# HadrienG2/grayscott

Measured on AMD Instinct MI355X. Metric: Mcells×steps/s and achieved HBM GB/s (% of roofline), 16384² f32 grid, higher is better.
Workload: dtype f32

## Files before the change

grayscott_amd/capi.py:

```python
from __future__ import annotations

import ctypes
import os

_HERE = os.path.dirname(os.path.abspath(__file__))
LIB_PATH = os.environ.get("GS_HIP_LIBRARY") or os.path.join(_HERE, "libgs_hip.so")

GS_OK = 0
GS_ERR_INVALID = -1
GS_ERR_HIP = -2
GS_ERR_RCCL = -3
GS_ERR_NO_DEVICE = -4
GS_ERR_UNSUPPORTED = -5
GS_ERR_NOMEM = -6

GS_MATH_STRICT, GS_MATH_FUSED = 0, 1
GS_KERNEL_AUTO, GS_KERNEL_SIMPLE, GS_KERNEL_STREAM, GS_KERNEL_TB, GS_KERNEL_LDS, GS_KERNEL_TILE, GS_KERNEL_WINDOW = 0, 1, 2, 3, 4, 5, 6
GS_BOUNDARY_CLIPPED, GS_BOUNDARY_ZERO_HALO, GS_BOUNDARY_PERIODIC, GS_BOUNDARY_NEUMANN = 0, 1, 2, 3
GS_UNIQUE_ID_BYTES = 128
GS_REGION_PAIRS_MAX = 1 << 25
GS_REGION_HIST_MAX = 1 << 25
GS_REGION_SPECTRUM_MAX = 1 << 25
GS_REGION_SPECTRUM_RECORDS_MAX = 1 << 27
GS_REGION_COMPONENTS_MAX = 1 << 20
# ... 26 lines not shown
    "gs_field_reduced_shape", "gs_field_download_reduced", "gs_field_download_reduced_async", "gs_field_colormap_reduced",
    "gs_fields_compare", "gs_members_compare", "gs_fields_copy", "gs_members_copy",
    "gs_members_set_active", "gs_members_get_active",
    "gs_members_set_noise", "gs_members_get_noise", "gs_members_clear_noise",
    "gs_fields_morphology", "gs_members_morphology",
    "gs_region_grid", "gs_fields_region_summaries", "gs_fields_region_morphology", "gs_fields_region_correlation",
    "gs_fields_region_histogram", "gs_fields_region_components", "gs_fields_region_compare", "gs_fields_region_spectrum",
    "gs_fields_correlation", "gs_members_correlation",
    "gs_spectrum_tables", "gs_fields_spectrum", "gs_members_spectrum",
    "gs_fields_components", "gs_members_components",
    "gs_field_component_list", "gs_members_component_list", "gs_component_list_view", "gs_component_list_destroy",
    "gs_fields_match", "gs_members_match", "gs_component_match_view", "gs_component_match_destroy",
    "gs_time_stats_create", "gs_time_stats_destroy", "gs_time_stats_reset", "gs_time_stats_accumulate", "gs_time_stats_samples",
    "gs_time_stats_result", "gs_time_stats_download",
    "gs_members_time_stats_create", "gs_members_time_stats_accumulate", "gs_members_time_stats_result",
    "gs_ctx_quiet_stats", "gs_ctx_quiet_edge_stats",
)


class GsError(RuntimeError):

    def __init__(self, code: int, message: str):
        super().__init__(f"gs_hip error {code}: {message}")
        self.code = code
        self.message = message


class GsParams(ctypes.Structure):

    _fields_ = [
        ("w", (ctypes.c_float * 3) * 3),
# ... 157 lines not shown
        "gs_timer_start": (i32, [vp]),
        "gs_timer_stop": (i32, [vp, P(f32)]),
        "gs_ctx_info": (i32, [vp, ctypes.c_char_p, ctypes.c_size_t, P(u64)]),
        "gs_host_alloc": (i32, [P(vp), u64]),
        "gs_host_free": (i32, [vp]),
        "gs_field_download_async": (i32, [vp, vp, vp]),
        "gs_download_wait": (i32, [vp]),
        "gs_ctx_get_tuned": (i32, [vp, u64, u64, P(i32), P(i32), P(i32), P(i32)]),
        "gs_ctx_set_tuned": (i32, [vp, u64, u64, i32, i32, i32, i32]),
        "gs_ctx_comm_info": (i32, [vp, P(i32), P(i32), P(i32)]),
        "gs_field_colormap": (i32, [vp, vp, f32, vp, i32, vp]),
        "gs_ctx_stats": (i32, [vp, P(GsStats)]),
        "gs_ctx_set_pass_timing": (i32, [vp, i32]),
        "gs_ctx_quiet_stats": (i32, [vp, P(u64)]),
        "gs_ctx_quiet_edge_stats": (i32, [vp, P(u64)]),
        "gs_field_mark_written": (i32, [vp, vp]),
        "gs_rccl_selftest": (i32, [i32, u64]),
        "gs_runtime_info": (i32, [i32, ctypes.c_char_p, ctypes.c_size_t]),
        "gs_fields_place": (i32, [vp, P(vp), i32, P(f32), P(f32)]),
        "gs_debug_place_stats": (i32, [vp, P(u64), P(u64)]),
        "gs_download_wait_but": (i32, [vp, i32]),
        "gs_debug_exchange_probe_create": (i32, [i32, i32, i32, u64, P(vp)]),
        "gs_debug_exchange_probe_run": (i32, [vp, P(f32), P(f32)]),
        "gs_debug_exchange_probe_destroy": (i32, [vp]),
        "gs_ensemble_create": (i32, [vp, P(vp), u64, u64, u64]),
        "gs_ensemble_destroy": (i32, [vp, vp]),
        "gs_ensemble_shape": (i32, [vp, P(u64), P(u64), P(u64)]),
        "gs_ensemble_set_params": (i32, [vp, vp, P(GsParams), u64]),
        "gs_ensemble_seed": (i32, [vp, vp]),
        "gs_ensemble_upload": (i32, [vp, vp, u64, u64, vp, vp]),
# ... 104 lines not shown
```

grayscott_amd/csrc/gs_api.cpp:

```cpp
#include "gs_internal.h"

namespace gsi {

bool is_pow2_or_zero(float w)
{
    if (w == 0.0f) return true;
    int e = 0;
    const float m = std::frexp(std::fabs(w), &e);
    return m == 0.5f;
}

int32_t check_math(const gs_params &p, int32_t math)
{
    if (math != GS_MATH_STRICT && math != GS_MATH_FUSED)
        return fail(GS_ERR_INVALID, "unknown math flavour %d", math);
    if (math == GS_MATH_FUSED)
        for (int i = 0; i < 3; ++i)
            for (int j = 0; j < 3; ++j)
                if (!is_pow2_or_zero(p.w[i][j]))
                    return fail(GS_ERR_UNSUPPORTED,
                                "GS_MATH_FUSED needs stencil weights that are 0 or a power of two "
                                "(w[%d][%d] = %g); use GS_MATH_STRICT", i, j, (double)p.w[i][j]);
    return GS_OK;
}
// ... 141 lines not shown
                    at.kind == GS_ATTACH_MAP ? "parameter-map" : (at.kind == GS_ATTACH_MASK ? "domain-mask" : "noise"));
    const char *name = nullptr;
    hipError_t e;
    switch (kernel) {
    case GS_KERNEL_TB:
        if (ctx->quiet.mode > 0 && !fused && at.kind == GS_ATTACH_NONE) {
            gs_ctx::QuietRt &qr = ctx->quiet;
            e = hipSuccess;
            for (int attempt = 0; attempt < 2; ++attempt) {
                GsQuiet q;
                q.in = qr.words + (size_t)qr.in_slot * qr.cap;
                q.out = qr.words + (size_t)(1 - qr.in_slot) * qr.cap;
                q.edge_skips = qr.words + 2 * qr.cap;
                q.skipped = qr.skipped;
                q.mode = qr.mode;
                q.cap = (int64_t)qr.cap;
                q.need = 0;
                q.launched = 0;
                q.edge_launched = 0;
                if (qr.mode == 1 && qr.words)
                    e = hipMemsetAsync(qr.words, 0, 2 * qr.cap * sizeof(uint32_t), stream);
                if (e == hipSuccess) e = gs_launch_tb_strict(a, fuse, stream, &name, at, &q);
                if (e != hipSuccess) break;
                if (q.need > (int64_t)qr.cap && qr.mode == 1) {
                    if (qr.words) {
                        GS_HIP(hipStreamSynchronize(stream));
                        uint64_t sum = 0;
                        GS_TRY(quiet_edge_skips(ctx, &sum));
                        qr.edge_skipped = sum;
                        GS_HIP(hipFree(qr.words));
                        qr.words = nullptr;
                        qr.cap = 0;
                    }
                    GS_HIP(hipMalloc(&qr.words, 3 * (size_t)q.need * sizeof(uint32_t)));
                    GS_HIP(hipMemset(qr.words, 0, 3 * (size_t)q.need * sizeof(uint32_t)));
                    qr.cap = (size_t)q.need;
                    if (!qr.skipped) {
                        GS_HIP(hipMalloc(&qr.skipped, (size_t)kQuietCounters * kQuietCounterStride * sizeof(unsigned long long)));
                        GS_HIP(hipMemset(qr.skipped, 0, (size_t)kQuietCounters * kQuietCounterStride * sizeof(unsigned long long)));
                    }
                    continue;
                }
                if (q.launched > 0) {
                    qr.launched += (uint64_t)q.launched;
                    qr.edge_launched += (uint64_t)q.edge_launched;
                    qr.passes++;
                    if (qr.mode == 3) qr.steady++;
                } else {
                    qr.refused = true;
                }
                break;
            }
            break;
        }
        e = fused ? gs_launch_tb_fused(a, fuse, stream, &name, at) : gs_launch_tb_strict(a, fuse, stream, &name, at);
        break;
    case GS_KERNEL_SIMPLE:
        e = fused ? gs_launch_simple_fused(a, stream, &name, at) : gs_launch_simple_strict(a, stream, &name, at);
        break;
    case GS_KERNEL_STREAM:
// ... 393 lines not shown
        for (int k = 0; k < 2; ++k) {
            if (b.done[k]) (void)hipEventDestroy(b.done[k]);
            if (b.halod[k]) (void)hipEventDestroy(b.halod[k]);
        }
    }
    if (!ctx->slabs.empty() && (ctx->win.words || ctx->win.planes[0] || ctx->win.desc) && hipSetDevice(ctx->slabs[0].device) == hipSuccess) {
        for (auto p : ctx->win.planes)
            if (p) (void)hipFree(p);
        if (ctx->win.words) (void)hipFree(ctx->win.words);
        if (ctx->win.desc) (void)hipFree(ctx->win.desc);
    }
    if (ctx->win.seen) (void)hipHostFree(ctx->win.seen);
    if (!ctx->slabs.empty() && (ctx->quiet.words || ctx->quiet.skipped) && hipSetDevice(ctx->slabs[0].device) == hipSuccess) {
        if (ctx->quiet.words) (void)hipFree(ctx->quiet.words);
        if (ctx->quiet.skipped) (void)hipFree(ctx->quiet.skipped);
    }
    if (ctx->graph_exec) (void)hipGraphExecDestroy(ctx->graph_exec);
    if (ctx->graph) (void)hipGraphDestroy(ctx->graph);
    if (ctx->band_join) (void)hipEventDestroy(ctx->band_join);
    const bool tuning = std::any_of(std::begin(ctx->tuner_of), std::end(ctx->tuner_of),
                                    [](const gs_ctx::TunerState &ts) { return !ts.tunings.empty(); });
    if (tuning && !ctx->slabs.empty() && hipSetDevice(ctx->slabs[0].device) == hipSuccess)
        for (auto &ts : ctx->tuner_of)
            for (auto &t : ts.tunings)
                for (auto e : t.events)
                    if (e) (void)hipEventDestroy(e);
    (void)hipGetLastError();
    delete ctx;
    return GS_OK;
}
// ... 18 lines not shown
                                            "set GS_RCCL_LIBRARY to the transport to use, or run one slab per process");
    }

    int ndev = 0;
    hipError_t e = hipGetDeviceCount(&ndev);
    if (e != hipSuccess || ndev == 0)
        return fail(GS_ERR_NO_DEVICE, "no HIP device available (%s)", hipGetErrorString(e));

    gs_ctx *ctx = new (std::nothrow) gs_ctx();
    if (!ctx) return fail(GS_ERR_NOMEM, "out of host memory");
    if (params) ctx->p = *params; else gs_default_params(&ctx->p);
    if (opts) ctx->o = *opts; else gs_default_options(&ctx->o);
    ctx->rank = rank;
    ctx->world = world;
    ctx->quiet.enabled = gs_env_int("GS_HIP_QUIET_UNITS", 1, 0, 1) != 0;
    int32_t st = check_math(ctx->p, ctx->o.math);
    if (st == GS_OK && ctx->o.cols_per_lane != 0 && ctx->o.cols_per_lane != 1 && ctx->o.cols_per_lane != 2 &&
        ctx->o.cols_per_lane != 4)
        st = fail(GS_ERR_INVALID, "cols_per_lane must be 0 (auto), 1, 2 or 4, not %d", ctx->o.cols_per_lane);
    if (st == GS_OK && (ctx->o.tile_shape < 0 || ctx->o.tile_shape > 3))
        st = fail(GS_ERR_INVALID, "tile_shape must be 0 (auto), 1 (32 x 64), 2 (16 x 64) or 3 (64 x 64), not %d", ctx->o.tile_shape);
    if (st == GS_OK && ctx->o.boundary != GS_BOUNDARY_CLIPPED && ctx->o.boundary != GS_BOUNDARY_ZERO_HALO &&
        ctx->o.boundary != GS_BOUNDARY_PERIODIC && ctx->o.boundary != GS_BOUNDARY_NEUMANN)
        st = fail(GS_ERR_INVALID, "unknown boundary rule %d", ctx->o.boundary);
    if (st == GS_OK && ctx->o.boundary == GS_BOUNDARY_PERIODIC) {
        if (world > 1 || n_local > 1)
            st = fail(GS_ERR_UNSUPPORTED, "the periodic boundary rule needs a single slab in a single process (got %d local "
                                          "slab(s), %d process(es))", n_local < 1 ? 1 : n_local, world);
        else if (ctx->o.kernel == GS_KERNEL_WINDOW || ctx->o.kernel == GS_KERNEL_LDS)
            st = fail(GS_ERR_UNSUPPORTED, "the periodic boundary rule has no form of the %s kernel",
// ... 207 lines not shown
    if (single && fuse > 1 && ctx->o.rows_per_block == 0 && !ctx->o.no_tune && !tuned_shape(ctx, u0, fuse))
        GS_TRY(tune_online(r, fuse));
    const int kk = tuned_shape(ctx, u0, fuse) && ctx->tuner().tuned.k > 0 && ctx->tuner().tuned.k <= fuse ? ctx->tuner().tuned.k : fuse;
    const int V = bands_for(ctx, u0, kk);
    if (ctx->o.use_graph && single && V == 1 && kk > 1) GS_TRY(replay_graph_batches(r, kk));
    gs_ctx::QuietRt &qr = ctx->quiet;
    const gs_params &pp = ctx->p;
    bool quiet = qr.enabled && single && V == 1 && !ctx->o.use_graph && !mapped && kk >= 2 && kk <= 4 &&
                 ctx->o.math == GS_MATH_STRICT && (ctx->o.boundary == GS_BOUNDARY_CLIPPED || ctx->o.boundary == GS_BOUNDARY_ZERO_HALO) &&
                 (ctx->o.kernel == GS_KERNEL_AUTO || ctx->o.kernel == GS_KERNEL_TB || ctx->o.kernel == GS_KERNEL_TILE ||
                  ctx->o.kernel == GS_KERNEL_WINDOW) &&
                 std::isfinite(pp.du) && std::isfinite(pp.dv) && std::isfinite(pp.feed) && std::isfinite(pp.kill) &&
                 std::isfinite(pp.feed + pp.kill) && std::isfinite(pp.dt);
    for (int i = 0; i < 9; ++i) quiet = quiet && std::isfinite(pp.w[i / 3][i % 3]);
    qr.refused = false;
    int quiet_pass = 0;
    const char *full_pass = nullptr;
    while (r.n < steps) {
        const int k = (steps - r.n) >= (uint64_t)kk ? kk : (int)(steps - r.n);
        if (quiet && k == kk && !qr.refused) {
            qr.mode = quiet_pass < 2 ? quiet_pass + 1 : 3;
            qr.in_slot = r.in;
            ++quiet_pass;
        }
        const int32_t st = r.advance(k == kk ? V : 1, k);
        qr.mode = 0;
        GS_TRY(st);
        if (k == kk) full_pass = ctx->last_kernel;
    }
    if (full_pass) ctx->last_kernel = full_pass;
    if (result_slot) *result_slot = r.in;
    return GS_OK;
}

}

// ... 100 lines not shown
int32_t gs_ctx_quiet_edge_stats(gs_ctx *ctx, uint64_t out[3])
{
    if (!ctx || !out) return fail(GS_ERR_INVALID, "null argument");
    GS_TRY(sync_all(ctx));
    out[0] = ctx->quiet.edge_launched;
    out[1] = out[2] = 0;
    if (ctx->quiet.skipped) {
        unsigned long long host[kQuietCounters * kQuietCounterStride];
        GS_HIP(hipSetDevice(ctx->slabs[0].device));
        GS_HIP(hipMemcpy(host, ctx->quiet.skipped, sizeof host, hipMemcpyDeviceToHost));
        for (int i = 0; i < kQuietCounters; ++i) out[2] += host[i * kQuietCounterStride + 2];
    }
    return gsi::quiet_edge_skips(ctx, &out[1]);
}

int32_t gs_ctx_info(const gs_ctx *ctx, char *kernel_name, size_t cap, uint64_t *launches)
{
    if (!ctx) return fail(GS_ERR_INVALID, "null context");
    if (kernel_name && cap) {
        const gs_ctx::Tuned &t = ctx->tuner().tuned;
        if (t.rpu > 0)
            std::snprintf(kernel_name, cap, "%s@%dx%d", ctx->last_kernel, t.rpu, t.split > 0 ? t.split : 1);
        else
            std::snprintf(kernel_name, cap, "%s", ctx->last_kernel);
    }
    if (launches) *launches = ctx->launches;
    return GS_OK;
}

}
// ... 1 lines not shown
```

grayscott_amd/csrc/gs_internal.h:

```cpp
#pragma once
#pragma GCC visibility push(default)
#include "../../include/gs_hip.h"
#pragma GCC visibility pop
#include "gs_kernels.h"
#include "gs_experiments.h"

#include <dlfcn.h>
#include <hip/hip_runtime.h>
#include <rccl/rccl.h>

#include <algorithm>
#include <cmath>
#include <cstdarg>
#include <cstdio>
#include <cstdlib>
#include <cstring>
#include <new>
#include <string>
#include <utility>
#include <vector>

namespace gsi {

extern thread_local std::string g_last_error;
// ... 128 lines not shown
        std::vector<Launch> launched;
        int32_t seq = 0;
        uint64_t fallbacks = 0;
        struct Image { gs_field *f; float *host; int32_t after_seq; int32_t factor; };
        std::vector<Image> images;
        int32_t *seen = nullptr;
    } win;
    int cu_count = 0;
    struct QuietRt {
        bool enabled = true;
        uint32_t *words = nullptr;
        size_t cap = 0;
        unsigned long long *skipped = nullptr;
        int mode = 0;
        int in_slot = 0;
        bool refused = false;
        uint64_t launched = 0, passes = 0, steady = 0;
        uint64_t edge_launched = 0;
        uint64_t edge_skipped = 0;
    } quiet;
    std::vector<struct gs_time_stats *> time_stats;
    struct Attached {
        int kind = GS_ATTACH_NONE;
        gs_field *plane[2] = {nullptr, nullptr};
        uint64_t gen = 0;
        gs_noise noise{};
    } attached;
    bool noisy() const { return attached.kind == GS_ATTACH_NOISE; }
    bool mapped() const { return attached.kind == GS_ATTACH_MAP; }
    bool masked() const { return attached.kind == GS_ATTACH_MASK; }
// ... 129 lines not shown
```

grayscott_amd/csrc/gs_kernels.h:

```cpp
#pragma once
#include <hip/hip_runtime.h>
#include <stdint.h>

constexpr int kGsResidentCells = 1536;
constexpr int kGsTileMaxSteps = 8;

struct GsStepArgs {
    const float *in_u, *in_v;
    float *out_u, *out_v;
    int32_t rows;
    int32_t cols;
    int32_t pitch;
    int32_t ra0, ra1, rb0, rb1;
    int32_t top_present, bottom_present;
    int32_t ghost;
    int32_t rows_per_unit;
    int32_t big_chunks, small_rpu;
    int32_t mid_chunks, tiny_rpu;
    int32_t bot_first;
    int32_t edge_split, edge_chunks;
    int32_t fast;
    int32_t cpl;
    int32_t allow_fair;
    int32_t edge_kinds;
    int32_t fair_from;
    int32_t xcd_m, xcd_first;
    int32_t zero_halo;
    float w[3][3];
    float du, dv, feed, feed_plus_kill, dt;
};
struct GsMapPlanes {
    const float *feed, *fpk;
};
struct GsMaskPlanes {
    const float *link;
};
constexpr uint32_t kQuietRest = 1, kQuietActive = 2;
constexpr int kQuietCounters = 64, kQuietCounterStride = 16;
struct GsQuiet {
    const uint32_t *in;
    uint32_t *out;
    uint32_t *edge_skips;
    unsigned long long *skipped;
    int32_t mode;
    int32_t pad;
    int64_t cap, need, launched, edge_launched;
};
struct GsNoiseArgs {
    uint32_t key[4];
    float sigma_u, sigma_v;
    uint32_t row0;
    uint32_t pad;
};
enum { GS_ATTACH_NONE = 0, GS_ATTACH_MAP = 1, GS_ATTACH_MASK = 2, GS_ATTACH_NOISE = 3, GS_ATTACH_KINDS = 4 };
struct GsAttached {
    int kind = GS_ATTACH_NONE;
    const float *plane[2] = {nullptr, nullptr};
    GsNoiseArgs noise = {};
};

constexpr int kGsWindowMaxNbr = 14;
// ... 220 lines not shown
```

grayscott_amd/csrc/gs_march.h:

```cpp
#pragma once

namespace {

__host__ __device__ constexpr int tb_sacrificial_lanes(int k, int cpl) { return (k + cpl - 1) / cpl; }
__host__ __device__ constexpr int tb_cols_per_wave(int k, int cpl) { return (64 - 2 * tb_sacrificial_lanes(k, cpl)) * cpl; }
static_assert(tb_cols_per_wave(4, 4) == 248 && tb_cols_per_wave(4, 1) == 56 && tb_cols_per_wave(3, 2) == 120, "");

template <int CPL>
struct RowQ {
    float u[CPL], v[CPL];
};
template <int CPL>
struct RowT {
    float u[CPL + 2], v[CPL + 2];
};

__device__ __forceinline__ int lane_id() { return (int)__builtin_amdgcn_mbcnt_hi(~0u, __builtin_amdgcn_mbcnt_lo(~0u, 0u)); }
__device__ __forceinline__ float shift_from_prev_lane(float own)
{
    return __builtin_bit_cast(float, __builtin_amdgcn_ds_bpermute(((lane_id() - 1) & 63) << 2, __builtin_bit_cast(int, own)));
}
__device__ __forceinline__ float shift_from_next_lane(float own)
{
    return __builtin_bit_cast(float, __builtin_amdgcn_ds_bpermute((((lane_id() - 1) & 63) << 2) + 8, __builtin_bit_cast(int, own)));
// ... 543 lines not shown
    if (a.xcd_m > 0 && block >= a.xcd_first) {
        const int per = 8 * a.xcd_m, r = block - a.xcd_first, g = r / per, o = r - g * per;
        if ((g + 1) * per <= (int)gridDim.x - a.xcd_first) block = a.xcd_first + g * per + (o & 7) * a.xcd_m + (o >> 3);
    }
    const int unit = FAIR && CPL == 1 ? wave * (int)gridDim.x + (int)blockIdx.x : block * WG + wave;
    const int rpu = a.rows_per_unit;
    const int small = a.small_rpu;
    const int rest_a = a.ra1 - a.ra0 - a.big_chunks * rpu;
    const int chunks_a = a.mid_chunks < 0 ? a.big_chunks + (rest_a + small - 1) / small
                                          : a.big_chunks + a.mid_chunks + (rest_a - a.mid_chunks * small + a.tiny_rpu - 1) / a.tiny_rpu;
    const int chunks_b = (a.rb1 - a.rb0 + rpu - 1) / rpu;
    const int chunks = chunks_a + chunks_b;
    const int er = ((strips - 1) * W + S * CPL >= a.cols && strips >= 2) ? 2 : 1;
    const int ne = 1 + er;
    const int es = a.edge_split == 2 ? 2 : 1;
    int chunk, strip, half = -1;
    if (strips <= ne) {
        if (unit >= chunks * strips * es) GS_TB_LEAVE;
        chunk = unit / (strips * es);
        const int rem = unit - chunk * strips * es;
        strip = rem / es;
        if (es == 2) half = rem - strip * es;
    } else if (unit < chunks * ne * es) {
        chunk = unit / (ne * es);
        const int rem = unit - chunk * ne * es, se = rem / es;
        if (es == 2) half = rem - se * es;
        strip = se == 0 ? 0 : strips - er + (se - 1);
    } else {
        const int ni = strips - ne, nec = es == 2 ? min(a.edge_chunks, chunks) : 0;
        int v = unit - chunks * ne * es;
        if (v < nec * ni * es) {
            chunk = v / (ni * es);
            const int rem = v - chunk * ni * es, si = rem / es;
            half = rem - si * es;
            strip = 1 + si;
        } else {
            v -= nec * ni * es;
            chunk = nec + v / ni;
            if (chunk >= chunks) GS_TB_LEAVE;
            strip = 1 + (v - (v / ni) * ni);
        }
    }
    int ur0, ur1;
    int row_chunk = -1;
    if (chunk < chunks_a) {
        const int bf = min(a.bot_first, chunks_a);
        const int cc = chunk < bf ? chunks_a - 1 - chunk : chunk - bf;
        row_chunk = cc;
        if (cc < a.big_chunks) {
            ur0 = a.ra0 + cc * rpu;
            ur1 = ur0 + rpu;
        } else if (a.mid_chunks < 0 || cc < a.big_chunks + a.mid_chunks) {
            ur0 = a.ra0 + a.big_chunks * rpu + (cc - a.big_chunks) * small;
// ... 1 lines not shown
        } else {
            ur0 = a.ra0 + a.big_chunks * rpu + a.mid_chunks * small + (cc - a.big_chunks - a.mid_chunks) * a.tiny_rpu;
            ur1 = min(ur0 + a.tiny_rpu, a.ra1);
        }
    } else {
        ur0 = a.rb0 + (chunk - chunks_a) * rpu;
        ur1 = min(ur0 + rpu, a.rb1);
    }
    const bool whole = half < 0 || ur1 - ur0 < 2;
    if (half >= 0) {
        const int hh = (ur1 - ur0 + 1) >> 1;
        if (half == 0) ur1 = min(ur0 + hh, ur1);
        else ur0 = ur0 + hh;
        if (ur0 >= ur1) GS_TB_LEAVE;
    }
    const bool left = strip == 0, right = (strip + 1) * W + S * CPL >= a.cols;
    const bool ends = (ur0 - K < 0 && !a.top_present) || (ur1 + K > a.rows && !a.bottom_present);
    const bool edge = left || right || ends;
#if defined(GS_TB_TRACE)
    unsigned long long ts[5] = {trace_now(), 0, 0, 0, 0};
    const unsigned long long cycles0 = __builtin_readcyclecounter();
#endif
    constexpr bool KINDS = (FAST & 1) && !GS_MATH_FUSED;
    if constexpr (QUIET) {
        typedef uint32_t word2 __attribute__((ext_vector_type(2)));
        if ((edge || half >= 0) && !a.zero_halo) {
            const int pos = row_chunk * strips + strip;
            const int nb = lane >> 1, part = lane & 1;
            int mine = 2 * pos + part, own = whole || part == half;
            asm volatile("" : "+v"(mine), "+v"(own));
            uint32_t word = kQuietRest;
            if (qa.mode >= 2) {
                const int rc = row_chunk + nb / 3 - 1, st = strip + nb % 3 - 1;
                if (lane < 18) {
                    if (rc >= 0 && rc < chunks_a && st >= 0 && st < strips) word = qa.in[2 * (rc * strips + st) + part];
                } else if (lane < 20 && qa.mode == 3 && own) {
                    word = qa.out[mine];
                }
            }
            bool rest = qa.mode >= 2 && __builtin_amdgcn_ballot_w64(lane < 18 && word != kQuietRest) == 0;
            const bool active = __builtin_amdgcn_ballot_w64(lane < 18 && nb == 4 && own && word == kQuietActive) != 0;
            int settled = qa.mode == 3 && __builtin_amdgcn_ballot_w64(lane >= 18 && word != kQuietRest) == 0;
            asm volatile("" : "+v"(settled));
            if (!rest && !active) {
                const int c = strip * W + (lane - S) * CPL;
                const int r0 = max(ur0 - K, 0), n = min(ur1 + K, a.rows) - r0;
                uint32_t differ = 0u;
#pragma unroll
                for (int e = 0; e < CPL; ++e) {
                    const ptrdiff_t at = (ptrdiff_t)r0 * a.pitch + min(max(c + e, 0), a.cols - 1);
                    const float *pu = a.in_u + at, *pv = a.in_v + at;
                    for (int r = 0; r < n; ++r, pu += a.pitch, pv += a.pitch)
                        differ |= (__builtin_bit_cast(uint32_t, *pu) ^ 0x3f800000u) | __builtin_bit_cast(uint32_t, *pv);
                }
                rest = __builtin_amdgcn_ballot_w64(differ != 0u) == 0;
            }
            if (rest && __builtin_amdgcn_readfirstlane(settled) != 0) {
                if (lane < 2 && own) qa.edge_skips[mine] += 1u;
                __builtin_amdgcn_endpgm();
            }
            if (lane < 2 && own) qa.out[mine] = rest ? kQuietRest : kQuietActive;
        }
        if (!edge) {
            const bool inner = half < 0 && row_chunk >= 0;
            const int pos = row_chunk * strips + strip;
            uint32_t *mine = inner ? qa.out + 2 * pos : nullptr;
            asm volatile("" : "+s"(mine));
            bool look = inner;
            int which = (strip == 1 || strip + 1 >= strips - er || row_chunk == 1 || row_chunk + 1 >= chunks_a - a.bot_first) ? 2 : 0;
            asm volatile("" : "+v"(which));
            if (inner && qa.mode >= 2) {
                const int nb = lane < 9 ? lane : 4;
                word2 w2 = {kQuietRest, kQuietRest};
                if (lane < 9) w2 = reinterpret_cast<const word2 *>(qa.in)[pos + (nb / 3 - 1) * strips + (nb % 3 - 1)];
                else if (lane == 9 && qa.mode == 3) w2 = reinterpret_cast<const word2 *>(qa.out)[pos];
                const uint32_t word = (w2.x == kQuietRest && w2.y == kQuietRest) ? kQuietRest
                                    : ((w2.x == kQuietActive || w2.y == kQuietActive) ? kQuietActive : 0u);
                if (qa.mode == 3 && __builtin_amdgcn_ballot_w64(word != kQuietRest) == 0) {
                    if (lane == 0)
                        (void)__hip_atomic_fetch_add(qa.skipped + ((int)blockIdx.x % kQuietCounters) * kQuietCounterStride + which, 1ull,
                                                     __ATOMIC_RELAXED, __HIP_MEMORY_SCOPE_AGENT);
                    return;
                }
                look = __builtin_amdgcn_ballot_w64(lane == 4 && word == kQuietActive) == 0;
            }
            unsigned long long dirty = 1;
            if (look)
                dirty = tb_march<K, 0, FAST, CPL, -1, FAIR, MAP, MASK, true>(a, ur0, ur1, strip, lane, mp, fb GS_TRACE_ARG);
            else
                tb_march<K, 0, FAST, CPL, -1, FAIR, MAP, MASK>(a, ur0, ur1, strip, lane, mp, fb GS_TRACE_ARG);
            if (mine && lane == 0) mine[0] = mine[1] = dirty ? kQuietActive : kQuietRest;
            return;
        }
    }
    if constexpr (PER) {
        if (!edge)
            tb_march<K, 0, FAST, CPL, -1, FAIR, MAP, MASK, false, NOISE>(a, ur0, ur1, strip, lane, mp, fb GS_TRACE_ARG, nz);
        else
            tb_march<K, 5, FAST, CPL, -1, FAIR, MAP, MASK, false, NOISE>(a, ur0, ur1, strip, lane, mp, fb GS_TRACE_ARG, nz);
    } else if constexpr (NEU) {
        if (!edge)
            tb_march<K, 0, FAST, CPL, -1, FAIR, MAP, MASK, false, NOISE>(a, ur0, ur1, strip, lane, mp, fb GS_TRACE_ARG, nz);
        else
            tb_march<K, 1, FAST, CPL, 3, FAIR, MAP, MASK, false, NOISE>(a, ur0, ur1, strip, lane, mp, fb GS_TRACE_ARG, nz);
    } else if (!edge)
        tb_march<K, 0, FAST, CPL, -1, FAIR, MAP, MASK, false, NOISE>(a, ur0, ur1, strip, lane, mp, fb GS_TRACE_ARG, nz);
    else if (a.zero_halo)
        tb_march<K, 1, FAST, CPL, 1, FAIR, MAP, MASK, false, NOISE>(a, ur0, ur1, strip, lane, mp, fb GS_TRACE_ARG, nz);
    else if (KINDS && a.edge_kinds && left && !right && !ends)
        tb_march<K, KINDS ? 2 : 1, FAST, CPL, 0, FAIR, MAP, MASK, false, NOISE>(a, ur0, ur1, strip, lane, mp, fb GS_TRACE_ARG, nz);
    else if (KINDS && a.edge_kinds && right && !left && !ends)
        tb_march<K, KINDS ? 3 : 1, FAST, CPL, 0, FAIR, MAP, MASK, false, NOISE>(a, ur0, ur1, strip, lane, mp, fb GS_TRACE_ARG, nz);
    else if (KINDS && a.edge_kinds && ends && !left && !right)
        tb_march<K, KINDS ? 4 : 1, FAST, CPL, 0, FAIR, MAP, MASK, false, NOISE>(a, ur0, ur1, strip, lane, mp, fb GS_TRACE_ARG, nz);
    else
        tb_march<K, 1, FAST, CPL, 0, FAIR, MAP, MASK, false, NOISE>(a, ur0, ur1, strip, lane, mp, fb GS_TRACE_ARG, nz);
    if constexpr (FAIR) { if (lane == 0) fb.progress[wave] = 0x7fffffff; }
#undef GS_TB_LEAVE
#if defined(GS_TB_TRACE)
    ts[4] = trace_now();
    const unsigned long long cycles = __builtin_readcyclecounter() - cycles0;
    if (lane == 0 && unit < kTraceUnits) {
        unsigned long long *rec = gs_trace_buf + (size_t)unit * kTraceWords;
        for (int i = 0; i < 5; ++i) rec[i] = ts[i];
        const unsigned hw = __builtin_amdgcn_s_getreg(4 | (0 << 6) | (31 << 11));
        const unsigned xcc = __builtin_amdgcn_s_getreg(20 | (0 << 6) | (3 << 11));
        rec[5] = ((unsigned long long)xcc << 32) | hw;
        rec[6] = ((unsigned long long)(unsigned)ur0 << 32) | (unsigned)((ur1 - ur0) | (edge ? 0x40000000 : 0));
        rec[7] = (cycles << 32) | (unsigned)strip;
    }
#endif
}

template <int K, int FAST, int CPL, int WG = 4>
// ... 67 lines not shown
```

grayscott_amd/csrc/gs_step_kernels.hip:

```cpp
#include "gs_kernels.h"
#include "gs_experiments.h"
#include <cstdio>
#include <cstdlib>
#include <mutex>

#ifndef GS_MATH_FUSED
#error "compile with -DGS_MATH_FUSED=0 or 1"
#endif
#ifndef GS_TB_OP_ONLY
#define GS_TB_OP_ONLY 0
#endif
#if GS_TB_OP_ONLY && GS_MATH_FUSED
#error "the fused build has no specialised variants"
#endif
#ifndef GS_TB_MAP_ONLY
#define GS_TB_MAP_ONLY 0
#endif
#if GS_TB_OP_ONLY && GS_TB_MAP_ONLY
#error "GS_TB_OP_ONLY and GS_TB_MAP_ONLY are translation units of their own"
#endif
#ifndef GS_TB_MASK_ONLY
#define GS_TB_MASK_ONLY 0
#endif
#if GS_TB_MASK_ONLY && (GS_TB_OP_ONLY || GS_TB_MAP_ONLY)
// ... 471 lines not shown
    auto chunk_rows = [&](long cc, long &r0, long &r1) {
        if (cc < big_chunks) { r0 = a.ra0 + cc * rpu; r1 = r0 + rpu; }
        else if (mid_chunks < 0 || cc < big_chunks + mid_chunks) { r0 = a.ra0 + big_chunks * rpu + (cc - big_chunks) * small; r1 = r0 + small < a.ra1 ? r0 + small : a.ra1; }
        else { r0 = a.ra0 + big_chunks * rpu + mid_chunks * small + (cc - big_chunks - mid_chunks) * tiny; r1 = r0 + tiny < a.ra1 ? r0 + tiny : a.ra1; }
    };
    long bot = 0, r0 = 0, r1 = 0;
    if (!a.bottom_present)
        for (; bot < chunks_a; ++bot) { chunk_rows(chunks_a - 1 - bot, r0, r1); if (!(r1 + k > a.rows)) break; }
    if (bot < 1 && chunks_a > 0) bot = 1;
    args.bot_first = (int32_t)bot;
    static const int split_env = gs_env_int("GS_HIP_EDGE_SPLIT", -1, 0, 1);
    const long er = ((strips - 1) * W + tb_sacrificial_lanes(k, cpl) * cpl >= a.cols && strips >= 2) ? 2 : 1, ne = 1 + er;
    bool split = 4 * chunks * strips <= 5 * slots && rpu >= 2;
    const bool quiet_ok = !GS_MATH_FUSED && quiet && quiet->mode >= 1 && quiet->mode <= 3 && at.kind == GS_ATTACH_NONE && per == 0 &&
                          fast == 15 && cpl == 2 && a.rb1 <= a.rb0 && !a.top_present && !a.bottom_present && rpu >= k && small >= k &&
                          tiny >= k && 2 * chunks * strips <= 0x7fffffffL;
    if (quiet_ok && quiet->mode == 3 && rpu >= 2) split = true;
    if (split_env >= 0) split = split_env != 0;
    long units = chunks * strips;
    args.edge_split = 1;
    args.edge_chunks = 0;
    if (split) {
        args.edge_split = 2;
        if (strips <= ne) {
            units = chunks * strips * 2;
        } else {
            const long nec = chunks_a > 0 ? (bot + 1 < chunks ? bot + 1 : chunks) : 0;
            args.edge_chunks = (int32_t)nec;
            units = chunks * ne * 2 + nec * (strips - ne) * 2 + (chunks - nec) * (strips - ne);
        }
    }
// ... 4 lines not shown
    static const int fair_from_env = gs_env_int("GS_HIP_FAIR_FROM", -1, 0, 256);
    args.fair_from = fair_from_env >= 0 ? fair_from_env : 0;
    void *kargs[] = {&args};
    if (fair_fn) {
        if (name) *name = names16[per][cpl == 1 ? 0 : 1][name_of(fast16)];
        return hipLaunchKernel(fair_fn, dim3((unsigned)((units + 15) / 16)), dim3(1024), kargs, 0, s);
    }
    const long blocks = (units + 3) / 4;
    if (blocks > 0x7fffffffL) return hipErrorInvalidConfiguration;
    static const int xcd_env = gs_env_int("GS_HIP_XCD_M", -1, 0, kGsXcdGroupMax);
    args.xcd_m = xcd_env >= 0 ? xcd_env : (units >= 2 * slots ? 16 : 0);
    args.xcd_first = (int32_t)(((chunks * ne * (args.edge_split == 2 ? 2 : 1) + 3) / 4 + 7) / 8 * 8);
#if !GS_MATH_FUSED
    if (quiet_ok) {
        if (const void *qfn = gs_tb_quiet_kernel_strict(k)) {
            quiet->need = 2 * chunks * strips;
            if (quiet->need <= quiet->cap && quiet->in && quiet->out && quiet->edge_skips && quiet->skipped) {
                GsQuiet q = *quiet;
                void *qargs[] = {&args, &q};
                quiet->launched = units;
                const long ends = bot + 1 < chunks ? bot + 1 : chunks, inner = strips <= ne ? 0 : (chunks - ends) * (strips - ne);
                quiet->edge_launched = split ? units - inner : chunks * strips - inner;
                return hipLaunchKernel(qfn, dim3((unsigned)blocks), dim3(256), qargs, 0, s);
            }
            if (quiet->mode == 1) return hipSuccess;
        }
    }
#endif
    return launch_attached(fn, blocks, args, at, s);
}

hipError_t GS_SUFFIX(gs_launch_lds)(const GsStepArgs &a, hipStream_t s, const char **name)
{
    if (name) *name = "lds-tile16/" GS_MATH_NAME;
    if (a.cols <= 0 || a.zero_halo >= 2) return hipErrorInvalidValue;
    const long chunks = ((long)(a.ra1 - a.ra0) + kLdsTileRows - 1) / kLdsTileRows +
                        ((long)(a.rb1 - a.rb0) + kLdsTileRows - 1) / kLdsTileRows;
    if (chunks <= 0) return hipSuccess;
// ... 247 lines not shown
```

grayscott_amd/simulation.py:

```python
from __future__ import annotations

import ctypes
import math
import os
from dataclasses import dataclass, field
from typing import Callable, List, Optional, Sequence, Tuple

import numpy as np

from . import capi
from .capi import GsError

STENCIL_WEIGHTS = ((0.25, 0.5, 0.25), (0.5, 0.0, 0.5), (0.25, 0.5, 0.25))

STENCILS = {
    "oono-puri": STENCIL_WEIGHTS,
    "5points": ((0.0, 1.0, 0.0), (1.0, 0.0, 1.0), (0.0, 1.0, 0.0)),
    "patrakarttunen": ((1 / 6, 4 / 6, 1 / 6), (4 / 6, 0.0, 4 / 6), (1 / 6, 4 / 6, 1 / 6)),
    "pretty": ((1.0, 1.0, 1.0), (1.0, 1.0, 1.0), (1.0, 1.0, 1.0)),
}


@dataclass
class Parameters:
# ... 127 lines not shown

    def stats(self) -> dict:
        st = capi.GsStats()
        capi.check(self._lib.gs_ctx_stats(self.handle, ctypes.byref(st)))
        return {name: getattr(st, name) for name, _ in capi.GsStats._fields_ if name != "reserved"}

    def quiet_stats(self) -> Tuple[int, int, int, int]:
        out = (ctypes.c_uint64 * 4)()
        capi.check(self._lib.gs_ctx_quiet_stats(self.handle, out))
        return int(out[0]), int(out[1]), int(out[2]), int(out[3])

    def quiet_edge_stats(self) -> Tuple[int, int, int]:
        out = (ctypes.c_uint64 * 3)()
        capi.check(self._lib.gs_ctx_quiet_edge_stats(self.handle, out))
        return int(out[0]), int(out[1]), int(out[2])

    def set_pass_timing(self, passes: int) -> None:
        capi.check(self._lib.gs_ctx_set_pass_timing(self.handle, passes))

    def info(self) -> Tuple[str, int]:
        buf = ctypes.create_string_buffer(64)
        n = ctypes.c_uint64(0)
        capi.check(self._lib.gs_ctx_info(self.handle, buf, 64, ctypes.byref(n)))
        return buf.value.decode(), int(n.value)

    def close(self) -> None:
        if self._h:
            self._lib.gs_ctx_destroy(self._h)
            self._h = ctypes.c_void_p()

# ... 2058 lines not shown
```

include/gs_hip.h:

```cpp
#ifndef GS_HIP_H
#define GS_HIP_H

#include <stddef.h>
#include <stdint.h>

#ifdef __cplusplus
extern "C" {
#endif

#define GS_ABI_VERSION 4

typedef enum gs_status {
    GS_OK = 0,
    GS_ERR_INVALID = -1,
    GS_ERR_HIP = -2,
    GS_ERR_RCCL = -3,
    GS_ERR_NO_DEVICE = -4,
    GS_ERR_UNSUPPORTED = -5,
    GS_ERR_NOMEM = -6
} gs_status;

typedef struct gs_params {
    float w[3][3];
    float du;
// ... 125 lines not shown
    uint64_t passes;
    uint64_t steps;
    uint64_t launches;
    uint64_t ghost_refreshes;
    uint64_t timed_passes;
    float halo_ms;
    float interior_ms;
    float halo_exposed_ms;
    float reserved;
    uint64_t window_fallbacks;
} gs_stats;
int32_t gs_ctx_stats(gs_ctx *ctx, gs_stats *out);
int32_t gs_ctx_set_pass_timing(gs_ctx *ctx, int32_t passes);
int32_t gs_ctx_quiet_stats(gs_ctx *ctx, uint64_t out[4]);
int32_t gs_ctx_quiet_edge_stats(gs_ctx *ctx, uint64_t out[3]);

int32_t gs_ctx_info(const gs_ctx *ctx, char *kernel_name, size_t cap, uint64_t *launches);

typedef struct gs_ensemble gs_ensemble;
int32_t gs_ensemble_create(gs_ctx *ctx, gs_ensemble **out, uint64_t members, uint64_t rows, uint64_t cols);
int32_t gs_ensemble_destroy(gs_ctx *ctx, gs_ensemble *e);
int32_t gs_ensemble_shape(const gs_ensemble *e, uint64_t *members, uint64_t *rows, uint64_t *cols);
int32_t gs_ensemble_set_params(gs_ctx *ctx, gs_ensemble *e, const gs_params *params, uint64_t count);
int32_t gs_ensemble_seed(gs_ctx *ctx, gs_ensemble *e);
int32_t gs_ensemble_upload(gs_ctx *ctx, gs_ensemble *e, uint64_t first, uint64_t count, const float *u, const float *v);
int32_t gs_ensemble_download(gs_ctx *ctx, gs_ensemble *e, uint64_t first, uint64_t count, int32_t species, float *host);
int32_t gs_ensemble_run(gs_ctx *ctx, gs_ensemble *e, uint64_t steps);

int32_t gs_members_set_active(gs_ctx *ctx, gs_ensemble *e, uint64_t first, uint64_t count, const uint8_t *active);
int32_t gs_members_get_active(gs_ctx *ctx, gs_ensemble *e, uint64_t first, uint64_t count, uint8_t *active, uint64_t *steps_taken,
// ... 154 lines not shown
```

Measured before the change: 4.906 million.

## Adaptively split active interior quiet units into row parts when few remain

```diff
diff --git a/grayscott_amd/capi.py b/grayscott_amd/capi.py
--- a/grayscott_amd/capi.py
+++ b/grayscott_amd/capi.py
@@ -64,7 +64,7 @@
     "gs_time_stats_create", "gs_time_stats_destroy", "gs_time_stats_reset", "gs_time_stats_accumulate", "gs_time_stats_samples",
     "gs_time_stats_result", "gs_time_stats_download",
     "gs_members_time_stats_create", "gs_members_time_stats_accumulate", "gs_members_time_stats_result",
-    "gs_ctx_quiet_stats", "gs_ctx_quiet_edge_stats",
+    "gs_ctx_quiet_stats", "gs_ctx_quiet_edge_stats", "gs_ctx_quiet_split_stats",
 )
 
 
@@ -252,6 +252,7 @@
         "gs_ctx_set_pass_timing": (i32, [vp, i32]),
         "gs_ctx_quiet_stats": (i32, [vp, P(u64)]),
         "gs_ctx_quiet_edge_stats": (i32, [vp, P(u64)]),
+        "gs_ctx_quiet_split_stats": (i32, [vp, P(u64)]),
         "gs_field_mark_written": (i32, [vp, vp]),
         "gs_rccl_selftest": (i32, [i32, u64]),
         "gs_runtime_info": (i32, [i32, ctypes.c_char_p, ctypes.c_size_t]),
diff --git a/grayscott_amd/csrc/gs_api.cpp b/grayscott_amd/csrc/gs_api.cpp
--- a/grayscott_amd/csrc/gs_api.cpp
+++ b/grayscott_amd/csrc/gs_api.cpp
@@ -179,10 +179,16 @@
                 q.edge_skips = qr.words + 2 * qr.cap;
                 q.skipped = qr.skipped;
                 q.mode = qr.mode;
+                q.slot = qr.split == 0 ? -1 : qr.pass % 3;
+                q.split = qr.mode != 3 || qr.split == 0 ? 0 : (qr.split > 0 ? (qr.pass >= 3 ? qr.split : 0) : (qr.pass >= 4 && !qr.dense ? 1 : 0));
+                q.limit = qr.split_units;
+                q.pad = 0;
+                q.hint = qr.pass >= 4 ? qr.hint : nullptr;
                 q.cap = (int64_t)qr.cap;
                 q.need = 0;
                 q.launched = 0;
                 q.edge_launched = 0;
+                q.part_launched = 0;
                 if (qr.mode == 1 && qr.words)
                     e = hipMemsetAsync(qr.words, 0, 2 * qr.cap * sizeof(uint32_t), stream);
                 if (e == hipSuccess) e = gs_launch_tb_strict(a, fuse, stream, &name, at, &q);
@@ -203,12 +209,17 @@
                     if (!qr.skipped) {
                         GS_HIP(hipMalloc(&qr.skipped, (size_t)kQuietCounters * kQuietCounterStride * sizeof(unsigned long long)));
                         GS_HIP(hipMemset(qr.skipped, 0, (size_t)kQuietCounters * kQuietCounterStride * sizeof(unsigned long long)));
+                        if (hipHostMalloc(reinterpret_cast<void **>(&qr.hint), sizeof(uint32_t), hipHostMallocDefault) == hipSuccess)
+                            *qr.hint = 0u;
+                        else
+                            qr.hint = nullptr;
                     }
                     continue;
                 }
                 if (q.launched > 0) {
                     qr.launched += (uint64_t)q.launched;
                     qr.edge_launched += (uint64_t)q.edge_launched;
+                    qr.part_launched += (uint64_t)q.part_launched;
                     qr.passes++;
                     if (qr.mode == 3) qr.steady++;
                 } else {
@@ -632,6 +643,7 @@
     if (!ctx->slabs.empty() && (ctx->quiet.words || ctx->quiet.skipped) && hipSetDevice(ctx->slabs[0].device) == hipSuccess) {
         if (ctx->quiet.words) (void)hipFree(ctx->quiet.words);
         if (ctx->quiet.skipped) (void)hipFree(ctx->quiet.skipped);
+        if (ctx->quiet.hint) (void)hipHostFree(ctx->quiet.hint);
     }
     if (ctx->graph_exec) (void)hipGraphExecDestroy(ctx->graph_exec);
     if (ctx->graph) (void)hipGraphDestroy(ctx->graph);
@@ -680,6 +692,9 @@
     ctx->rank = rank;
     ctx->world = world;
     ctx->quiet.enabled = gs_env_int("GS_HIP_QUIET_UNITS", 1, 0, 1) != 0;
+    ctx->quiet.split = gs_env_int("GS_HIP_QUIET_SPLIT", -1, 0, 4);
+    if (ctx->quiet.split == 1 || ctx->quiet.split == 3) ctx->quiet.split = -1;
+    ctx->quiet.split_units = (uint32_t)gs_env_int("GS_HIP_QUIET_SPLIT_UNITS", kQuietSplitUnits, 0, 1 << 28);
     int32_t st = check_math(ctx->p, ctx->o.math);
     if (st == GS_OK && ctx->o.cols_per_lane != 0 && ctx->o.cols_per_lane != 1 && ctx->o.cols_per_lane != 2 &&
         ctx->o.cols_per_lane != 4)
@@ -917,12 +932,14 @@
                  std::isfinite(pp.feed + pp.kill) && std::isfinite(pp.dt);
     for (int i = 0; i < 9; ++i) quiet = quiet && std::isfinite(pp.w[i / 3][i % 3]);
     qr.refused = false;
+    qr.dense = qr.hint && *static_cast<volatile uint32_t *>(qr.hint) > 2ull * qr.split_units;
     int quiet_pass = 0;
     const char *full_pass = nullptr;
     while (r.n < steps) {
         const int k = (steps - r.n) >= (uint64_t)kk ? kk : (int)(steps - r.n);
         if (quiet && k == kk && !qr.refused) {
             qr.mode = quiet_pass < 2 ? quiet_pass + 1 : 3;
+            qr.pass = quiet_pass;
             qr.in_slot = r.in;
             ++quiet_pass;
         }
@@ -1053,6 +1070,23 @@
     return gsi::quiet_edge_skips(ctx, &out[1]);
 }
 
+int32_t gs_ctx_quiet_split_stats(gs_ctx *ctx, uint64_t out[4])
+{
+    if (!ctx || !out) return fail(GS_ERR_INVALID, "null argument");
+    GS_TRY(sync_all(ctx));
+    out[0] = out[1] = out[2] = 0;
+    out[3] = ctx->quiet.part_launched;
+    if (ctx->quiet.skipped) {
+        unsigned long long host[kQuietCounters * kQuietCounterStride];
+        GS_HIP(hipSetDevice(ctx->slabs[0].device));
+        GS_HIP(hipMemcpy(host, ctx->quiet.skipped, sizeof host, hipMemcpyDeviceToHost));
+        out[0] = host[3 * kQuietCounterStride + kQuietSumAt];
+        out[1] = host[4 * kQuietCounterStride + kQuietSumAt];
+        for (int i = 0; i < kQuietCounters; ++i) out[2] += host[i * kQuietCounterStride + kQuietPartsAt] & 0xffffffffull;
+    }
+    return GS_OK;
+}
+
 int32_t gs_ctx_info(const gs_ctx *ctx, char *kernel_name, size_t cap, uint64_t *launches)
 {
     if (!ctx) return fail(GS_ERR_INVALID, "null context");
diff --git a/grayscott_amd/csrc/gs_internal.h b/grayscott_amd/csrc/gs_internal.h
--- a/grayscott_amd/csrc/gs_internal.h
+++ b/grayscott_amd/csrc/gs_internal.h
@@ -166,6 +166,12 @@
         unsigned long long *skipped = nullptr;
         int mode = 0;
         int in_slot = 0;
+        int pass = 0;
+        int split = -1;
+        uint32_t split_units = 0;
+        uint64_t part_launched = 0;
+        uint32_t *hint = nullptr;
+        bool dense = false;
         bool refused = false;
         uint64_t launched = 0, passes = 0, steady = 0;
         uint64_t edge_launched = 0;
diff --git a/grayscott_amd/csrc/gs_kernels.h b/grayscott_amd/csrc/gs_kernels.h
--- a/grayscott_amd/csrc/gs_kernels.h
+++ b/grayscott_amd/csrc/gs_kernels.h
@@ -1,6 +1,7 @@
 #pragma once
 #include <hip/hip_runtime.h>
 #include <stdint.h>
+#include "gs_parts.h"
 
 constexpr int kGsResidentCells = 1536;
 constexpr int kGsTileMaxSteps = 8;
@@ -37,14 +38,20 @@
 };
 constexpr uint32_t kQuietRest = 1, kQuietActive = 2;
 constexpr int kQuietCounters = 64, kQuietCounterStride = 16;
+constexpr int kQuietCountAt = 8;
+constexpr int kQuietPartsAt = 11;
+constexpr int kQuietSplitUnits = 1024;
+constexpr int kQuietSumAt = 12;
 struct GsQuiet {
     const uint32_t *in;
     uint32_t *out;
     uint32_t *edge_skips;
     unsigned long long *skipped;
     int32_t mode;
-    int32_t pad;
-    int64_t cap, need, launched, edge_launched;
+    int32_t slot, split;
+    uint32_t limit, pad;
+    uint32_t *hint;
+    int64_t cap, need, launched, edge_launched, part_launched;
 };
 struct GsNoiseArgs {
     uint32_t key[4];
diff --git a/grayscott_amd/csrc/gs_march.h b/grayscott_amd/csrc/gs_march.h
--- a/grayscott_amd/csrc/gs_march.h
+++ b/grayscott_amd/csrc/gs_march.h
@@ -581,6 +581,32 @@
     const int er = ((strips - 1) * W + S * CPL >= a.cols && strips >= 2) ? 2 : 1;
     const int ne = 1 + er;
     const int es = a.edge_split == 2 ? 2 : 1;
+    int nparts = 1, mypart = 0;
+    bool splits = false;
+    if constexpr (QUIET) {
+        if (qa.slot >= 0) {
+            const int next = qa.slot == 2 ? 0 : qa.slot + 1, prev = qa.slot == 0 ? 2 : qa.slot - 1;
+            if (qa.split >= 2) {
+                nparts = qa.split;
+            } else if (qa.split == 1) {
+                const uint32_t sum = __builtin_amdgcn_readfirstlane(
+                    *reinterpret_cast<const uint32_t *>(qa.skipped + qa.slot * kQuietCounterStride + kQuietSumAt));
+                nparts = sum <= qa.limit ? 4 : (sum <= 2 * (unsigned long long)qa.limit ? 2 : 1);
+            }
+            if (blockIdx.x == 0 && wave == 0) {
+                unsigned long long *line = qa.skipped + lane * kQuietCounterStride;
+                int sum_at = next * kQuietCounterStride + kQuietSumAt;
+                asm volatile("" : "+v"(sum_at));
+                (void)__hip_atomic_fetch_add(reinterpret_cast<uint32_t *>(qa.skipped + sum_at),
+                                             *reinterpret_cast<const uint32_t *>(line + kQuietCountAt + prev), __ATOMIC_RELAXED,
+                                             __HIP_MEMORY_SCOPE_AGENT);
+                *reinterpret_cast<uint32_t *>(line + kQuietCountAt + next) = 0u;
+                *reinterpret_cast<uint32_t *>(qa.skipped + prev * kQuietCounterStride + kQuietSumAt) = 0u;
+                if (nparts > 1) qa.skipped[(nparts == 2 ? 3 : 4) * kQuietCounterStride + kQuietSumAt] += 1ull;
+                if (qa.hint) *qa.hint = *reinterpret_cast<const uint32_t *>(qa.skipped + qa.slot * kQuietCounterStride + kQuietSumAt);
+            }
+        }
+    }
     int chunk, strip, half = -1;
     if (strips <= ne) {
         if (unit >= chunks * strips * es) GS_TB_LEAVE;
@@ -604,6 +630,18 @@
         } else {
             v -= nec * ni * es;
             chunk = nec + v / ni;
+            if constexpr (QUIET) {
+                splits = true;
+                if (chunk >= chunks) {
+                    if (nparts == 1) GS_TB_LEAVE;
+                    v -= (chunks - nec) * ni;
+                    const int at = v / (kQuietMaxParts - 1);
+                    mypart = 1 + (v - at * (kQuietMaxParts - 1));
+                    v = at;
+                    chunk = nec + v / ni;
+                    if (mypart >= nparts) GS_TB_LEAVE;
+                }
+            }
             if (chunk >= chunks) GS_TB_LEAVE;
             strip = 1 + (v - (v / ni) * ni);
         }
@@ -635,6 +673,18 @@
         else ur0 = ur0 + hh;
         if (ur0 >= ur1) GS_TB_LEAVE;
     }
+    if constexpr (QUIET) {
+        nparts = __builtin_amdgcn_readfirstlane(nparts);
+        mypart = __builtin_amdgcn_readfirstlane(mypart);
+        splits = splits && nparts > 1;
+        if (splits) {
+            int r0, r1;
+            gs_part_rows(ur1 - ur0, nparts, mypart, r0, r1);
+            ur1 = ur0 + r1;
+            ur0 = ur0 + r0;
+            if (ur0 >= ur1) GS_TB_LEAVE;
+        }
+    }
     const bool left = strip == 0, right = (strip + 1) * W + S * CPL >= a.cols;
     const bool ends = (ur0 - K < 0 && !a.top_present) || (ur1 + K > a.rows && !a.bottom_present);
     const bool edge = left || right || ends;
@@ -645,6 +695,7 @@
     constexpr bool KINDS = (FAST & 1) && !GS_MATH_FUSED;
     if constexpr (QUIET) {
         typedef uint32_t word2 __attribute__((ext_vector_type(2)));
+        typedef uint32_t word4 __attribute__((ext_vector_type(4)));
         if ((edge || half >= 0) && !a.zero_halo) {
             const int pos = row_chunk * strips + strip;
             const int nb = lane >> 1, part = lane & 1;
@@ -653,11 +704,14 @@
             uint32_t word = kQuietRest;
             if (qa.mode >= 2) {
                 const int rc = row_chunk + nb / 3 - 1, st = strip + nb % 3 - 1;
+                word2 w2 = {kQuietRest, kQuietRest};
                 if (lane < 18) {
-                    if (rc >= 0 && rc < chunks_a && st >= 0 && st < strips) word = qa.in[2 * (rc * strips + st) + part];
+                    if (rc >= 0 && rc < chunks_a && st >= 0 && st < strips) w2 = reinterpret_cast<const word2 *>(qa.in)[2 * (rc * strips + st) + part];
                 } else if (lane < 20 && qa.mode == 3 && own) {
-                    word = qa.out[mine];
-                }
+                    w2 = reinterpret_cast<const word2 *>(qa.out)[mine];
+                }
+                word = (w2.x == kQuietRest && w2.y == kQuietRest) ? kQuietRest
+                     : ((w2.x == kQuietActive || w2.y == kQuietActive) ? kQuietActive : 0u);
             }
             bool rest = qa.mode >= 2 && __builtin_amdgcn_ballot_w64(lane < 18 && word != kQuietRest) == 0;
             const bool active = __builtin_amdgcn_ballot_w64(lane < 18 && nb == 4 && own && word == kQuietActive) != 0;
@@ -680,38 +734,74 @@
                 if (lane < 2 && own) qa.edge_skips[mine] += 1u;
                 __builtin_amdgcn_endpgm();
             }
-            if (lane < 2 && own) qa.out[mine] = rest ? kQuietRest : kQuietActive;
+            if (lane < 2 && own) {
+                const uint32_t w = rest ? kQuietRest : kQuietActive;
+                reinterpret_cast<word2 *>(qa.out)[mine] = word2{w, w};
+            }
         }
         if (!edge) {
             const bool inner = half < 0 && row_chunk >= 0;
             const int pos = row_chunk * strips + strip;
-            uint32_t *mine = inner ? qa.out + 2 * pos : nullptr;
+            const int nown = splits ? kQuietMaxParts / nparts : kQuietMaxParts;
+            uint32_t *mine = inner ? reinterpret_cast<uint32_t *>(reinterpret_cast<uintptr_t>(qa.out + 4 * pos + mypart * nown) |
+                                                                  (uintptr_t)(nown == 4 ? 0 : (nown == 2 ? 1 : 2)))
+                                   : nullptr;
             asm volatile("" : "+s"(mine));
             bool look = inner;
             int which = (strip == 1 || strip + 1 >= strips - er || row_chunk == 1 || row_chunk + 1 >= chunks_a - a.bot_first) ? 2 : 0;
             asm volatile("" : "+v"(which));
             if (inner && qa.mode >= 2) {
                 const int nb = lane < 9 ? lane : 4;
-                word2 w2 = {kQuietRest, kQuietRest};
-                if (lane < 9) w2 = reinterpret_cast<const word2 *>(qa.in)[pos + (nb / 3 - 1) * strips + (nb % 3 - 1)];
-                else if (lane == 9 && qa.mode == 3) w2 = reinterpret_cast<const word2 *>(qa.out)[pos];
-                const uint32_t word = (w2.x == kQuietRest && w2.y == kQuietRest) ? kQuietRest
-                                    : ((w2.x == kQuietActive || w2.y == kQuietActive) ? kQuietActive : 0u);
+                word4 w4 = {kQuietRest, kQuietRest, kQuietRest, kQuietRest};
+                if (lane < 9) {
+                    w4 = reinterpret_cast<const word4 *>(qa.in)[pos + (nb / 3 - 1) * strips + (nb % 3 - 1)];
+                } else if (lane == 9 && qa.mode == 3) {
+                    if (nown == 4) {
+                        w4 = reinterpret_cast<const word4 *>(qa.out)[pos];
+                    } else if (nown == 2) {
+                        const word2 w2 = reinterpret_cast<const word2 *>(qa.out)[2 * pos + mypart];
+                        w4 = word4{w2.x, w2.y, w2.x, w2.y};
+                    } else {
+                        const uint32_t w = qa.out[4 * pos + mypart];
+                        w4 = word4{w, w, w, w};
+                    }
+                }
+                const uint32_t word = (w4.x == kQuietRest && w4.y == kQuietRest && w4.z == kQuietRest && w4.w == kQuietRest) ? kQuietRest
+                                    : ((w4.x == kQuietActive || w4.y == kQuietActive || w4.z == kQuietActive || w4.w == kQuietActive) ? kQuietActive : 0u);
                 if (qa.mode == 3 && __builtin_amdgcn_ballot_w64(word != kQuietRest) == 0) {
-                    if (lane == 0)
+                    if (lane == 0 && mypart == 0)
                         (void)__hip_atomic_fetch_add(qa.skipped + ((int)blockIdx.x % kQuietCounters) * kQuietCounterStride + which, 1ull,
                                                      __ATOMIC_RELAXED, __HIP_MEMORY_SCOPE_AGENT);
                     return;
                 }
                 look = __builtin_amdgcn_ballot_w64(lane == 4 && word == kQuietActive) == 0;
+                if (qa.slot >= 0 && lane == 0) {
+                    unsigned long long *line = qa.skipped + ((int)blockIdx.x % kQuietCounters) * kQuietCounterStride;
+                    (void)__hip_atomic_fetch_add(reinterpret_cast<uint32_t *>(line + kQuietCountAt + qa.slot), (uint32_t)nown,
+                                                 __ATOMIC_RELAXED, __HIP_MEMORY_SCOPE_AGENT);
+                    if (mypart > 0)
+                        (void)__hip_atomic_fetch_add(reinterpret_cast<uint32_t *>(line + kQuietPartsAt), 1u, __ATOMIC_RELAXED,
+                                                     __HIP_MEMORY_SCOPE_AGENT);
+                }
             }
             unsigned long long dirty = 1;
             if (look)
                 dirty = tb_march<K, 0, FAST, CPL, -1, FAIR, MAP, MASK, true>(a, ur0, ur1, strip, lane, mp, fb GS_TRACE_ARG);
             else
                 tb_march<K, 0, FAST, CPL, -1, FAIR, MAP, MASK>(a, ur0, ur1, strip, lane, mp, fb GS_TRACE_ARG);
-            if (mine && lane == 0) mine[0] = mine[1] = dirty ? kQuietActive : kQuietRest;
+            if (mine && lane == 0) {
+                const uint32_t w = dirty ? kQuietActive : kQuietRest;
+                const uintptr_t at = reinterpret_cast<uintptr_t>(mine);
+                uint32_t *first = reinterpret_cast<uint32_t *>(at & ~(uintptr_t)3);
+                if ((at & 3) == 0) *reinterpret_cast<word4 *>(first) = word4{w, w, w, w};
+                else if ((at & 3) == 1) *reinterpret_cast<word2 *>(first) = word2{w, w};
+                else *first = w;
+            }
+#if defined(GS_TB_TRACE)
+            goto traced;
+#else
             return;
+#endif
         }
     }
     if constexpr (PER) {
@@ -739,6 +829,7 @@
     if constexpr (FAIR) { if (lane == 0) fb.progress[wave] = 0x7fffffff; }
 #undef GS_TB_LEAVE
 #if defined(GS_TB_TRACE)
+traced: __attribute__((unused));
     ts[4] = trace_now();
     const unsigned long long cycles = __builtin_readcyclecounter() - cycles0;
     if (lane == 0 && unit < kTraceUnits) {
diff --git a/grayscott_amd/csrc/gs_parts.h b/grayscott_amd/csrc/gs_parts.h
--- /dev/null
+++ b/grayscott_amd/csrc/gs_parts.h
@@ -0,0 +1,31 @@
+#pragma once
+
+#if defined(__HIPCC__) || defined(__CUDACC__)
+#define GS_PARTS_HD __host__ __device__
+#else
+#define GS_PARTS_HD
+#endif
+
+constexpr int kQuietMaxParts = 4;
+
+GS_PARTS_HD inline void gs_part_rows(int rows, int P, int p, int &r0, int &r1)
+{
+    r0 = 0;
+    r1 = rows;
+    if (P >= 2) {
+        const int hh = (rows + 1) >> 1;
+        if (p < P / 2) r1 = hh;
+        else r0 = hh;
+    }
+    if (P == 4) {
+        const int qh = (r1 - r0 + 1) >> 1;
+        if ((p & 1) == 0) r1 = r0 + qh;
+        else r0 = r0 + qh;
+    }
+}
+
+GS_PARTS_HD inline long gs_part_waves(long chunks, long strips, long ne, long nec)
+{
+    if (strips <= ne || chunks <= nec) return 0;
+    return (chunks - nec) * (strips - ne) * (kQuietMaxParts - 1);
+}
diff --git a/grayscott_amd/csrc/gs_step_kernels.hip b/grayscott_amd/csrc/gs_step_kernels.hip
--- a/grayscott_amd/csrc/gs_step_kernels.hip
+++ b/grayscott_amd/csrc/gs_step_kernels.hip
@@ -509,7 +509,7 @@
     bool split = 4 * chunks * strips <= 5 * slots && rpu >= 2;
     const bool quiet_ok = !GS_MATH_FUSED && quiet && quiet->mode >= 1 && quiet->mode <= 3 && at.kind == GS_ATTACH_NONE && per == 0 &&
                           fast == 15 && cpl == 2 && a.rb1 <= a.rb0 && !a.top_present && !a.bottom_present && rpu >= k && small >= k &&
-                          tiny >= k && 2 * chunks * strips <= 0x7fffffffL;
+                          tiny >= k && 2 * kQuietMaxParts * chunks * strips <= 0x7fffffffL;
     if (quiet_ok && quiet->mode == 3 && rpu >= 2) split = true;
     if (split_env >= 0) split = split_env != 0;
     long units = chunks * strips;
@@ -544,14 +544,20 @@
 #if !GS_MATH_FUSED
     if (quiet_ok) {
         if (const void *qfn = gs_tb_quiet_kernel_strict(k)) {
-            quiet->need = 2 * chunks * strips;
+            quiet->need = kQuietMaxParts * chunks * strips;
             if (quiet->need <= quiet->cap && quiet->in && quiet->out && quiet->edge_skips && quiet->skipped) {
                 GsQuiet q = *quiet;
                 void *qargs[] = {&args, &q};
-                quiet->launched = units;
+                long part_waves = 0;
+                if (q.mode == 3 && q.slot >= 0 && q.split != 0 && args.edge_split == 2) part_waves = gs_part_waves(chunks, strips, ne, args.edge_chunks);
+                if (part_waves == 0) q.split = 0;
+                quiet->part_launched = part_waves;
+                const long qblocks = (units + part_waves + 3) / 4;
+                if (qblocks > 0x7fffffffL) return hipErrorInvalidConfiguration;
+                quiet->launched = units + part_waves;
                 const long ends = bot + 1 < chunks ? bot + 1 : chunks, inner = strips <= ne ? 0 : (chunks - ends) * (strips - ne);
                 quiet->edge_launched = split ? units - inner : chunks * strips - inner;
-                return hipLaunchKernel(qfn, dim3((unsigned)blocks), dim3(256), qargs, 0, s);
+                return hipLaunchKernel(qfn, dim3((unsigned)qblocks), dim3(256), qargs, 0, s);
             }
             if (quiet->mode == 1) return hipSuccess;
         }
diff --git a/grayscott_amd/simulation.py b/grayscott_amd/simulation.py
--- a/grayscott_amd/simulation.py
+++ b/grayscott_amd/simulation.py
@@ -165,6 +165,11 @@
         out = (ctypes.c_uint64 * 3)()
         capi.check(self._lib.gs_ctx_quiet_edge_stats(self.handle, out))
         return int(out[0]), int(out[1]), int(out[2])
+
+    def quiet_split_stats(self) -> Tuple[int, int, int, int]:
+        out = (ctypes.c_uint64 * 4)()
+        capi.check(self._lib.gs_ctx_quiet_split_stats(self.handle, out))
+        return int(out[0]), int(out[1]), int(out[2]), int(out[3])
 
     def set_pass_timing(self, passes: int) -> None:
         capi.check(self._lib.gs_ctx_set_pass_timing(self.handle, passes))
diff --git a/include/gs_hip.h b/include/gs_hip.h
--- a/include/gs_hip.h
+++ b/include/gs_hip.h
@@ -163,6 +163,7 @@
 int32_t gs_ctx_set_pass_timing(gs_ctx *ctx, int32_t passes);
 int32_t gs_ctx_quiet_stats(gs_ctx *ctx, uint64_t out[4]);
 int32_t gs_ctx_quiet_edge_stats(gs_ctx *ctx, uint64_t out[3]);
+int32_t gs_ctx_quiet_split_stats(gs_ctx *ctx, uint64_t out[4]);
 
 int32_t gs_ctx_info(const gs_ctx *ctx, char *kernel_name, size_t cap, uint64_t *launches);
 
```

New measurement: 6.209 million, median of 6. +26.6%, better.
